# EthanD11/RS-VIO

Measured on AMD Instinct MI355X. Metric: stereo frames/sec (tracker+BA) on 752×480 EuRoC stream; BA ms/iter at window=10, higher is better.
Workload: dtype f32 (tracker) / f64 (BA)

## Files before the change

rs-vio_amd/csrc/pyramid.hip:

```cpp
#include "pyramid.hpp"

namespace rsvio {

namespace {

constexpr int TW = 64;
constexpr int TH = 8;
constexpr int STRIP_COLS = 320;
constexpr size_t LDS_CAP = 64 << 10;

__device__ __forceinline__ float triangle_kernel(float x) {
    float ax = fabsf(x);
    return ax < 1.0f ? 1.0f - ax : 0.0f;
}

__global__ void make_taps_kernel(TapTable tab, int n_entries) {
    int e = blockIdx.x * blockDim.x + threadIdx.x;
    if (e >= n_entries) return;
    int in_len = tab.ent_in_len[e];
    int out_len = tab.ent_out_len[e];
    int o = tab.ent_out_idx[e];
    float ratio = (float)in_len / (float)out_len;
    float sratio = ratio < 1.0f ? 1.0f : ratio;
    float support = 1.0f * sratio;
    float inputc = ((float)o + 0.5f) * ratio;
    long long left = (long long)floorf(inputc - support);
    if (left < 0) left = 0;
    if (left > (long long)in_len - 1) left = in_len - 1;
    long long right = (long long)ceilf(inputc + support);
    if (right < left + 1) right = left + 1;
    if (right > (long long)in_len) right = in_len;
    inputc = inputc - 0.5f;
    int cnt = (int)(right - left);
    float* w = tab.weights + (size_t)e * tab.max_taps;
    float sum = 0.0f;
    for (int k = 0; k < cnt; ++k) {
        float wv = triangle_kernel(((float)(left + k) - inputc) / sratio);
        w[k] = wv;
        sum += wv;
    }
    for (int k = 0; k < cnt; ++k) w[k] = w[k] / sum;
    tab.left[e] = (int)left;
    tab.count[e] = cnt;
}

__global__ __launch_bounds__(256) void pyramid_kernel(PyrLaunch L, PyrIO io) {
    extern __shared__ uint32_t smem[];
    const int img = blockIdx.y;
    {
        const int fb = (int)blockIdx.x - (L.copy_blocks + L.tile_start[L.levels]);
        if (fb >= 0) {
            if (img == 0 && fb < io.fast_cells) {
                const uint8_t* s0 = io.psrc ? io.psrc : io.src[0];
                fast_cell(s0, io.fg, fb, nullptr, nullptr, 0, io.fast_pt, io.fast_aff,
                          reinterpret_cast<uint8_t*>(smem));
            }
            return;
        }
    }
    const uint8_t* __restrict__ src = io.psrc ? io.psrc + (size_t)img * L.w * L.h : io.src[img];
    uint8_t* __restrict__ dst_base = io.psrc ? io.pdst + (size_t)img * L.pyr_bytes : io.dst[img];
    int b = blockIdx.x;
    const bool aligned = ((reinterpret_cast<uintptr_t>(src) | reinterpret_cast<uintptr_t>(dst_base)) & 15) == 0;
    if (b < L.copy_blocks) {
        const size_t tot = (size_t)L.w * L.h;
        if (!aligned) {
            for (size_t i = (size_t)b * blockDim.x + threadIdx.x; i < tot; i += (size_t)L.copy_blocks * blockDim.x)
                dst_base[i] = src[i];
            return;
        }
        const size_t n16 = tot / 16;
        const uint4* s4 = reinterpret_cast<const uint4*>(src);
        uint4* d4 = reinterpret_cast<uint4*>(dst_base);
        for (size_t i = (size_t)b * blockDim.x + threadIdx.x; i < n16; i += (size_t)L.copy_blocks * blockDim.x)
            d4[i] = s4[i];
        size_t tail0 = n16 * 16;
        if (b == 0)
            for (size_t i = tail0 + threadIdx.x; i < tot; i += blockDim.x) dst_base[i] = src[i];
        return;
    }
    b -= L.copy_blocks;
    int lev = 1;
    while (lev < L.levels - 1 && b >= L.tile_start[lev + 1]) ++lev;
    b -= L.tile_start[lev];
    const int nw = (int)level_w(L.w, lev), nh = (int)level_h(L.h, lev);
    const int tw = L.tile_w[lev], th = L.tile_h[lev];
    const int tiles_x = (nw + tw - 1) / tw;
    const int tx = b % tiles_x, ty = b / tiles_x;
    const int ox0 = tx * tw, ox1 = min(ox0 + tw, nw);
    const int oy0 = ty * th, oy1 = min(oy0 + th, nh);
    const int rows = oy1 - oy0, cols_out = ox1 - ox0;
    const int hx = L.hx_ent[lev], vy = L.vy_ent[lev];
    const TapTable& T = L.tab;
    const int xl = T.left[hx + ox0];
    const int xr = T.left[hx + ox1 - 1] + T.count[hx + ox1 - 1];
    const int yl = T.left[vy + oy0];
    const int yr = T.left[vy + oy1 - 1] + T.count[vy + oy1 - 1];
    const int ncols = xr - xl, nrows = yr - yl;
    const int xa = xl & ~3, xoff = xl - xa;
    const int pd = (xr - xa + 3) >> 2;
    const bool direct = (L.direct >> lev) & 1;
    uint8_t* strip = reinterpret_cast<uint8_t*>(smem);
    if (!direct) {
        if (aligned && (L.w & 3) == 0) {
            const uint32_t* s32 = reinterpret_cast<const uint32_t*>(src);
            const int wd = (int)(L.w >> 2);
            for (int idx = threadIdx.x; idx < nrows * pd; idx += blockDim.x) {
                const int r = idx / pd, d = idx - r * pd;
                smem[idx] = s32[(size_t)(yl + r) * wd + (xa >> 2) + d];
            }
        } else {
            for (int idx = threadIdx.x; idx < nrows * pd * 4; idx += blockDim.x) {
                const int r = idx / (pd * 4), c = idx - r * pd * 4;
                strip[idx] = (xa + c < (int)L.w) ? src[(size_t)(yl + r) * L.w + xa + c] : 0;
            }
        }
    }
    float* tmp = reinterpret_cast<float*>(smem + (direct ? 0 : nrows * pd));
    __syncthreads();
    for (int idx = threadIdx.x; idx < rows * ncols; idx += blockDim.x) {
        const int r = idx / ncols, c = idx - r * ncols;
        const int e = vy + oy0 + r;
        const int vl = T.left[e], vc = T.count[e];
        const float* __restrict__ vw = T.weights + (size_t)e * T.max_taps;
        float acc = 0.0f;
        if (!direct) {
            const uint8_t* col = strip + (vl - yl) * pd * 4 + xoff + c;
            for (int k = 0; k < vc; ++k) acc += (float)col[k * pd * 4] * vw[k];
        } else {
            const uint8_t* __restrict__ col = src + (size_t)vl * L.w + xl + c;
            for (int k = 0; k < vc; k += 8) {
                float px[8];
#pragma unroll
                for (int u = 0; u < 8; ++u) px[u] = (k + u < vc) ? (float)col[(size_t)(k + u) * L.w] : 0.0f;
#pragma unroll
                for (int u = 0; u < 8; ++u)
                    if (k + u < vc) acc += px[u] * vw[k + u];
            }
        }
        tmp[r * ncols + c] = acc;
    }
    __syncthreads();
    uint8_t* __restrict__ dst = dst_base + level_offset(L.w, L.h, lev);
    for (int idx = threadIdx.x; idx < rows * cols_out; idx += blockDim.x) {
        const int r = idx / cols_out, c = idx - r * cols_out;
        const int e = hx + ox0 + c;
        const int hl = T.left[e] - xl, hc = T.count[e];
        const float* __restrict__ hw = T.weights + (size_t)e * T.max_taps;
        const float* __restrict__ row = tmp + r * ncols + hl;
        float acc = 0.0f;
        for (int k = 0; k < hc; ++k) acc += row[k] * hw[k];
        float cl = acc < 0.0f ? 0.0f : (acc > 255.0f ? 255.0f : acc);
        dst[(size_t)(oy0 + r) * nw + ox0 + c] = (uint8_t)roundf(cl);
    }
}

}

void PyramidPlan::init(int w_, int h_, int levels_) {
    w = w_;
    h = h_;
    levels = levels_;
    if (levels < 1 || levels > kMaxLevels) throw std::invalid_argument("levels must be in [1, 8]");
    if (w < 16 || h < 16) throw std::invalid_argument("image too small");
    std::vector<int> in_len, out_len, out_idx;
    float max_ratio = 1.0f;
    memset(&launch, 0, sizeof(launch));
    for (int i = 1; i < levels; ++i) {
        int nw = (int)level_w(w, i), nh = (int)level_h(h, i);
        if (nw < 1 || nh < 1) throw std::invalid_argument("too many levels for image size");
        launch.hx_ent[i] = (int)in_len.size();
        for (int o = 0; o < nw; ++o) { in_len.push_back(w); out_len.push_back(nw); out_idx.push_back(o); }
        launch.vy_ent[i] = (int)in_len.size();
        for (int o = 0; o < nh; ++o) { in_len.push_back(h); out_len.push_back(nh); out_idx.push_back(o); }
        float rx = (float)w / nw, ry = (float)h / nh;
        max_ratio = std::max(max_ratio, std::max(rx, ry));
        launch.tile_h[i] = std::max(1, std::min(TH, (int)(16.0f / ry)));
        launch.tile_w[i] = std::max(1, std::min(TW, (int)std::floor((STRIP_COLS - 2.0f * rx - 4.0f) / rx)));
    }
    n_entries = (int)in_len.size();
    max_taps = (int)std::ceil(2.0f * max_ratio) + 4;
    int tiles = 0;
    for (int i = 1; i < levels; ++i) {
        launch.tile_start[i] = tiles;
        int nw = (int)level_w(w, i), nh = (int)level_h(h, i);
        tiles += ((nw + launch.tile_w[i] - 1) / launch.tile_w[i]) * ((nh + launch.tile_h[i] - 1) / launch.tile_h[i]);
    }
    launch.tile_start[levels] = tiles;
    launch.copy_blocks = std::max(1, (int)(((size_t)w * h / 16 + 255) / 256 / 4));
    total_blocks = launch.copy_blocks + tiles;
    launch.w = (uint32_t)w;
    launch.h = (uint32_t)h;
    launch.levels = levels;
    launch.pyr_bytes = level_offset(w, h, levels);
    if (n_entries > 0) {
        i_in.alloc(n_entries); i_out.alloc(n_entries); i_idx.alloc(n_entries);
        d_left.alloc(n_entries); d_count.alloc(n_entries);
        d_w.alloc((size_t)n_entries * max_taps);
        RSVIO_HIP(hipMemcpy(i_in.p, in_len.data(), sizeof(int) * n_entries, hipMemcpyHostToDevice));
        RSVIO_HIP(hipMemcpy(i_out.p, out_len.data(), sizeof(int) * n_entries, hipMemcpyHostToDevice));
        RSVIO_HIP(hipMemcpy(i_idx.p, out_idx.data(), sizeof(int) * n_entries, hipMemcpyHostToDevice));
        TapTable t;
        t.left = d_left.p; t.count = d_count.p; t.weights = d_w.p; t.max_taps = max_taps;
        t.ent_in_len = i_in.p; t.ent_out_len = i_out.p; t.ent_out_idx = i_idx.p;
        hipLaunchKernelGGL(make_taps_kernel, dim3((n_entries + 255) / 256), dim3(256), 0, 0, t, n_entries);
        RSVIO_HIP(hipGetLastError());
        RSVIO_HIP(hipDeviceSynchronize());
        launch.tab = t;
        std::vector<int> left(n_entries), count(n_entries);
        RSVIO_HIP(hipMemcpy(left.data(), d_left.p, sizeof(int) * n_entries, hipMemcpyDeviceToHost));
        RSVIO_HIP(hipMemcpy(count.data(), d_count.p, sizeof(int) * n_entries, hipMemcpyDeviceToHost));
        for (int i = 1; i < levels; ++i) {
            const int nw = (int)level_w(w, i), nh = (int)level_h(h, i);
            const int tw = launch.tile_w[i], th = launch.tile_h[i];
            size_t strip = 0, vert = 0;
            for (int ox0 = 0; ox0 < nw; ox0 += tw) {
                const int ox1 = std::min(ox0 + tw, nw);
                const int xl = left[launch.hx_ent[i] + ox0];
                const int xr = left[launch.hx_ent[i] + ox1 - 1] + count[launch.hx_ent[i] + ox1 - 1];
                const size_t pd = (size_t)(xr - (xl & ~3) + 3) / 4;
                for (int oy0 = 0; oy0 < nh; oy0 += th) {
                    const int oy1 = std::min(oy0 + th, nh);
                    const int yl = left[launch.vy_ent[i] + oy0];
                    const int yr = left[launch.vy_ent[i] + oy1 - 1] + count[launch.vy_ent[i] + oy1 - 1];
                    strip = std::max(strip, 4 * pd * (size_t)(yr - yl));
                    vert = std::max(vert, 4 * (size_t)(oy1 - oy0) * (size_t)(xr - xl));
                }
            }
            if (vert > LDS_CAP) throw std::invalid_argument("image too wide for the pyramid tile");
            if (strip + vert > LDS_CAP) launch.direct |= 1u << i;
            lds_bytes = std::max(lds_bytes, ((launch.direct >> i) & 1) ? vert : strip + vert);
        }
    }
}

void PyramidPlan::enqueue(const PyrIO& io, int n_img, hipStream_t s) const {
    if (n_img <= 0) return;
    if (n_img > (io.psrc ? 65535 : kMaxPyrIO)) throw std::invalid_argument("too many images per pyramid launch");
    const size_t lds = io.fast_cells > 0 ? std::max(lds_bytes, (size_t)io.fg.g * io.fg.g) : lds_bytes;
    hipLaunchKernelGGL(pyramid_kernel, dim3(total_blocks + std::max(io.fast_cells, 0), n_img), dim3(256), lds, s,
                       launch, io);
    RSVIO_HIP(hipGetLastError());
}

void PyramidPlan::enqueue(const uint8_t* d_imgs, int n_img, uint8_t* d_pyrs, hipStream_t s) const {
    for (int i0 = 0; i0 < n_img; i0 += 65535) {
        PyrIO io{};
        io.psrc = d_imgs + (size_t)i0 * w * h;
        io.pdst = d_pyrs + (size_t)i0 * pyr_bytes();
        enqueue(io, std::min(65535, n_img - i0), s);
    }
}

}
```

rs-vio_amd/csrc/pyramid.hpp:

```cpp
#pragma once
#include <algorithm>
#include <cmath>
#include <cstring>
#include <stdexcept>
#include <vector>

#include "common.hpp"
#include "fast.hpp"

namespace rsvio {

constexpr int kMaxLevels = 8;

struct TapTable {
    int* left = nullptr;
    int* count = nullptr;
    float* weights = nullptr;
    int max_taps = 0;
    const int* ent_in_len = nullptr;
    const int* ent_out_len = nullptr;
    const int* ent_out_idx = nullptr;
};

struct PyrLaunch {
    uint32_t w, h;
    int levels;
    size_t pyr_bytes;
    int copy_blocks;
    int tile_start[kMaxLevels + 1];
    int tile_w[kMaxLevels];
    int tile_h[kMaxLevels];
    uint32_t direct;
    int hx_ent[kMaxLevels];
    int vy_ent[kMaxLevels];
    TapTable tab;
};

constexpr int kMaxPyrIO = 8;
struct PyrIO {
    const uint8_t* src[kMaxPyrIO];
    uint8_t* dst[kMaxPyrIO];
    const uint8_t* psrc;
    uint8_t* pdst;
    int fast_cells;
    GridGeom fg;
    int4* fast_pt;
    float* fast_aff;
};

struct PyramidPlan {
    int w = 0, h = 0, levels = 0;
    int n_entries = 0, max_taps = 0, total_blocks = 0;
    size_t lds_bytes = 0;
    PyrLaunch launch;
    DevBuf<int> i_in, i_out, i_idx, d_left, d_count;
    DevBuf<float> d_w;
    void init(int w, int h, int levels);
    size_t pyr_bytes() const { return level_offset(w, h, levels); }
    void enqueue(const uint8_t* d_imgs, int n_img, uint8_t* d_pyrs, hipStream_t s) const;
    void enqueue(const PyrIO& io, int n_img, hipStream_t s) const;
};

}
```

Before: 4859.

## Stage tap weights in LDS and vectorize vertical pass over packed pixels

Reworks the pyramid downsample kernel. Tap tables are cached in LDS per tile, and tile bounds are computed inline rather than read from global memory. The vertical pass now processes four packed bytes per thread from the strip, strided index division is replaced with incremental DivStep counters, and global loads are unrolled to raise memory-level parallelism. The tile height default grows from 8 to 12 and the LDS sizing is updated, which raises LDS use per block and may lower occupancy.

```diff
diff --git a/rs-vio_amd/csrc/pyramid.hip b/rs-vio_amd/csrc/pyramid.hip
--- a/rs-vio_amd/csrc/pyramid.hip
+++ b/rs-vio_amd/csrc/pyramid.hip
@@ -4,22 +4,29 @@
 
 namespace {
 
+constexpr int NT = 256;
 constexpr int TW = 64;
-constexpr int TH = 8;
+#ifndef RSVIO_PYR_TH
+#define RSVIO_PYR_TH 12
+#endif
+constexpr int TH = RSVIO_PYR_TH;
 constexpr int STRIP_COLS = 320;
 constexpr size_t LDS_CAP = 64 << 10;
+constexpr int SU = 8;
+constexpr int WU = 4;
+static_assert(TW + TH <= NT, "one thread per tap row of a tile");
 
 __device__ __forceinline__ float triangle_kernel(float x) {
     float ax = fabsf(x);
     return ax < 1.0f ? 1.0f - ax : 0.0f;
 }
 
-__global__ void make_taps_kernel(TapTable tab, int n_entries) {
-    int e = blockIdx.x * blockDim.x + threadIdx.x;
-    if (e >= n_entries) return;
-    int in_len = tab.ent_in_len[e];
-    int out_len = tab.ent_out_len[e];
-    int o = tab.ent_out_idx[e];
+struct TapSpan {
+    int left, count;
+    float inputc, sratio;
+};
+
+__device__ __forceinline__ TapSpan tap_span(int in_len, int out_len, int o) {
     float ratio = (float)in_len / (float)out_len;
     float sratio = ratio < 1.0f ? 1.0f : ratio;
     float support = 1.0f * sratio;
@@ -31,18 +38,42 @@
     if (right < left + 1) right = left + 1;
     if (right > (long long)in_len) right = in_len;
     inputc = inputc - 0.5f;
-    int cnt = (int)(right - left);
+    return TapSpan{(int)left, (int)(right - left), inputc, sratio};
+}
+
+__global__ void make_taps_kernel(TapTable tab, int n_entries) {
+    int e = blockIdx.x * blockDim.x + threadIdx.x;
+    if (e >= n_entries) return;
+    const TapSpan sp = tap_span(tab.ent_in_len[e], tab.ent_out_len[e], tab.ent_out_idx[e]);
     float* w = tab.weights + (size_t)e * tab.max_taps;
     float sum = 0.0f;
-    for (int k = 0; k < cnt; ++k) {
-        float wv = triangle_kernel(((float)(left + k) - inputc) / sratio);
+    for (int k = 0; k < sp.count; ++k) {
+        float wv = triangle_kernel(((float)((long long)sp.left + k) - sp.inputc) / sp.sratio);
         w[k] = wv;
         sum += wv;
     }
-    for (int k = 0; k < cnt; ++k) w[k] = w[k] / sum;
-    tab.left[e] = (int)left;
-    tab.count[e] = cnt;
-}
+    for (int k = 0; k < sp.count; ++k) w[k] = w[k] / sum;
+    tab.left[e] = sp.left;
+    tab.count[e] = sp.count;
+}
+
+struct DivStep {
+    int q, r, dq, dr, n;
+    __device__ __forceinline__ explicit DivStep(int n_) : n(n_) {
+        q = (int)threadIdx.x / n;
+        r = (int)threadIdx.x - q * n;
+        dq = NT / n;
+        dr = NT - dq * n;
+    }
+    __device__ __forceinline__ void next() {
+        q += dq;
+        r += dr;
+        if (r >= n) {
+            r -= n;
+            ++q;
+        }
+    }
+};
 
 __global__ __launch_bounds__(256) void pyramid_kernel(PyrLaunch L, PyrIO io) {
     extern __shared__ uint32_t smem[];
@@ -92,62 +123,135 @@
     const int rows = oy1 - oy0, cols_out = ox1 - ox0;
     const int hx = L.hx_ent[lev], vy = L.vy_ent[lev];
     const TapTable& T = L.tab;
-    const int xl = T.left[hx + ox0];
-    const int xr = T.left[hx + ox1 - 1] + T.count[hx + ox1 - 1];
-    const int yl = T.left[vy + oy0];
-    const int yr = T.left[vy + oy1 - 1] + T.count[vy + oy1 - 1];
+    const int tid = threadIdx.x;
+    const TapSpan sx0 = tap_span((int)L.w, nw, ox0), sx1 = tap_span((int)L.w, nw, ox1 - 1);
+    const TapSpan sy0 = tap_span((int)L.h, nh, oy0), sy1 = tap_span((int)L.h, nh, oy1 - 1);
+    const int xl = sx0.left, xr = sx1.left + sx1.count;
+    const int yl = sy0.left, yr = sy1.left + sy1.count;
     const int ncols = xr - xl, nrows = yr - yl;
-    const int xa = xl & ~3, xoff = xl - xa;
+    const bool direct = (L.direct >> lev) & 1;
+    const int xa = direct ? xl : (xl & ~3);
     const int pd = (xr - xa + 3) >> 2;
-    const bool direct = (L.direct >> lev) & 1;
-    uint8_t* strip = reinterpret_cast<uint8_t*>(smem);
+    const int tc = L.tap_cap[lev];
+    const int ne = cols_out + rows, nwt = ne * tc;
+    float* tmp = reinterpret_cast<float*>(smem);
+    uint32_t* strip32 = smem + rows * 4 * pd;
+    uint8_t* strip = reinterpret_cast<uint8_t*>(strip32);
+    int* s_left = reinterpret_cast<int*>(strip32 + (direct ? 0 : nrows * pd));
+    int* s_count = s_left + ne;
+    float* s_w = reinterpret_cast<float*>(s_count + ne);
+    int t_left = 0, t_count = 0;
+    if (tid < ne) {
+        const int e = tid < cols_out ? hx + ox0 + tid : vy + oy0 + (tid - cols_out);
+        t_left = T.left[e];
+        t_count = T.count[e];
+    }
+    float wv[WU];
+    DivStep jk(tc);
+#pragma unroll
+    for (int u = 0; u < WU; ++u) {
+        const int j = jk.q;
+        const int e = j < cols_out ? hx + ox0 + j : vy + oy0 + (j - cols_out);
+        wv[u] = (tid + u * NT < nwt) ? T.weights[(size_t)e * T.max_taps + jk.r] : 0.0f;
+        jk.next();
+    }
     if (!direct) {
         if (aligned && (L.w & 3) == 0) {
-            const uint32_t* s32 = reinterpret_cast<const uint32_t*>(src);
-            const int wd = (int)(L.w >> 2);
-            for (int idx = threadIdx.x; idx < nrows * pd; idx += blockDim.x) {
-                const int r = idx / pd, d = idx - r * pd;
-                smem[idx] = s32[(size_t)(yl + r) * wd + (xa >> 2) + d];
+            const uint32_t* __restrict__ s32 = reinterpret_cast<const uint32_t*>(src);
+            const int wd = (int)(L.w >> 2), n = nrows * pd;
+            DivStep rd(pd);
+            for (int base = tid; base < n; base += NT * SU) {
+                uint32_t v[SU];
+#pragma unroll
+                for (int u = 0; u < SU; ++u) {
+                    v[u] = (base + u * NT < n) ? s32[(size_t)(yl + rd.q) * wd + (xa >> 2) + rd.r] : 0u;
+                    rd.next();
+                }
+#pragma unroll
+                for (int u = 0; u < SU; ++u)
+                    if (base + u * NT < n) strip32[base + u * NT] = v[u];
             }
         } else {
-            for (int idx = threadIdx.x; idx < nrows * pd * 4; idx += blockDim.x) {
-                const int r = idx / (pd * 4), c = idx - r * pd * 4;
-                strip[idx] = (xa + c < (int)L.w) ? src[(size_t)(yl + r) * L.w + xa + c] : 0;
-            }
-        }
-    }
-    float* tmp = reinterpret_cast<float*>(smem + (direct ? 0 : nrows * pd));
+            const int n = nrows * pd * 4;
+            DivStep rc(pd * 4);
+            for (int base = tid; base < n; base += NT * SU) {
+                uint8_t v[SU];
+#pragma unroll
+                for (int u = 0; u < SU; ++u) {
+                    v[u] = (base + u * NT < n && xa + rc.r < (int)L.w) ? src[(size_t)(yl + rc.q) * L.w + xa + rc.r]
+                                                                       : (uint8_t)0;
+                    rc.next();
+                }
+#pragma unroll
+                for (int u = 0; u < SU; ++u)
+                    if (base + u * NT < n) strip[base + u * NT] = v[u];
+            }
+        }
+    }
+    if (tid < ne) {
+        s_left[tid] = t_left;
+        s_count[tid] = t_count;
+    }
+#pragma unroll
+    for (int u = 0; u < WU; ++u)
+        if (tid + u * NT < nwt) s_w[tid + u * NT] = wv[u];
+    for (int idx = tid + WU * NT; idx < nwt; idx += NT) {
+        const int j = jk.q;
+        const int e = j < cols_out ? hx + ox0 + j : vy + oy0 + (j - cols_out);
+        s_w[idx] = T.weights[(size_t)e * T.max_taps + jk.r];
+        jk.next();
+    }
     __syncthreads();
-    for (int idx = threadIdx.x; idx < rows * ncols; idx += blockDim.x) {
-        const int r = idx / ncols, c = idx - r * ncols;
-        const int e = vy + oy0 + r;
-        const int vl = T.left[e], vc = T.count[e];
-        const float* __restrict__ vw = T.weights + (size_t)e * T.max_taps;
-        float acc = 0.0f;
-        if (!direct) {
-            const uint8_t* col = strip + (vl - yl) * pd * 4 + xoff + c;
-            for (int k = 0; k < vc; ++k) acc += (float)col[k * pd * 4] * vw[k];
-        } else {
-            const uint8_t* __restrict__ col = src + (size_t)vl * L.w + xl + c;
-            for (int k = 0; k < vc; k += 8) {
-                float px[8];
-#pragma unroll
-                for (int u = 0; u < 8; ++u) px[u] = (k + u < vc) ? (float)col[(size_t)(k + u) * L.w] : 0.0f;
-#pragma unroll
-                for (int u = 0; u < 8; ++u)
-                    if (k + u < vc) acc += px[u] * vw[k + u];
-            }
-        }
-        tmp[r * ncols + c] = acc;
+    if (!direct) {
+        DivStep rd(pd);
+        for (int idx = tid; idx < rows * pd; idx += NT, rd.next()) {
+            const int r = rd.q, d = rd.r, j = cols_out + r;
+            const int vc = s_count[j];
+            const float* vw = s_w + j * tc;
+            const uint32_t* col = strip32 + (s_left[j] - yl) * pd + d;
+            float a0 = 0.0f, a1 = 0.0f, a2 = 0.0f, a3 = 0.0f;
+            for (int k = 0; k < vc; ++k) {
+                const uint32_t p = col[k * pd];
+                const float wk = vw[k];
+                a0 += (float)(p & 0xffu) * wk;
+                a1 += (float)((p >> 8) & 0xffu) * wk;
+                a2 += (float)((p >> 16) & 0xffu) * wk;
+                a3 += (float)(p >> 24) * wk;
+            }
+            float* o = tmp + (r * pd + d) * 4;
+            o[0] = a0;
+            o[1] = a1;
+            o[2] = a2;
+            o[3] = a3;
+        }
+    } else {
+        for (int r = 0; r < rows; ++r) {
+            const int j = cols_out + r;
+            const int vl = s_left[j], vc = s_count[j];
+            const float* vw = s_w + j * tc;
+            for (int c = tid; c < ncols; c += NT) {
+                const uint8_t* __restrict__ col = src + (size_t)vl * L.w + xl + c;
+                float acc = 0.0f;
+                for (int k = 0; k < vc; k += 8) {
+                    float px[8];
+#pragma unroll
+                    for (int u = 0; u < 8; ++u) px[u] = (k + u < vc) ? (float)col[(size_t)(k + u) * L.w] : 0.0f;
+#pragma unroll
+                    for (int u = 0; u < 8; ++u)
+                        if (k + u < vc) acc += px[u] * vw[k + u];
+                }
+                tmp[r * pd * 4 + c] = acc;
+            }
+        }
     }
     __syncthreads();
     uint8_t* __restrict__ dst = dst_base + level_offset(L.w, L.h, lev);
-    for (int idx = threadIdx.x; idx < rows * cols_out; idx += blockDim.x) {
-        const int r = idx / cols_out, c = idx - r * cols_out;
-        const int e = hx + ox0 + c;
-        const int hl = T.left[e] - xl, hc = T.count[e];
-        const float* __restrict__ hw = T.weights + (size_t)e * T.max_taps;
-        const float* __restrict__ row = tmp + r * ncols + hl;
+    DivStep rc(cols_out);
+    for (int idx = tid; idx < rows * cols_out; idx += NT, rc.next()) {
+        const int r = rc.q, c = rc.r;
+        const int hc = s_count[c];
+        const float* hw = s_w + c * tc;
+        const float* row = tmp + r * pd * 4 + (s_left[c] - xa);
         float acc = 0.0f;
         for (int k = 0; k < hc; ++k) acc += row[k] * hw[k];
         float cl = acc < 0.0f ? 0.0f : (acc > 255.0f ? 255.0f : acc);
@@ -175,7 +279,7 @@
         for (int o = 0; o < nh; ++o) { in_len.push_back(h); out_len.push_back(nh); out_idx.push_back(o); }
         float rx = (float)w / nw, ry = (float)h / nh;
         max_ratio = std::max(max_ratio, std::max(rx, ry));
-        launch.tile_h[i] = std::max(1, std::min(TH, (int)(16.0f / ry)));
+        launch.tile_h[i] = std::max(1, std::min(TH, (int)(2.0f * TH / ry)));
         launch.tile_w[i] = std::max(1, std::min(TW, (int)std::floor((STRIP_COLS - 2.0f * rx - 4.0f) / rx)));
     }
     n_entries = (int)in_len.size();
@@ -213,23 +317,28 @@
         for (int i = 1; i < levels; ++i) {
             const int nw = (int)level_w(w, i), nh = (int)level_h(h, i);
             const int tw = launch.tile_w[i], th = launch.tile_h[i];
-            size_t strip = 0, vert = 0;
+            int tc = 1;
+            for (int e = launch.hx_ent[i]; e < launch.hx_ent[i] + nw + nh; ++e) tc = std::max(tc, count[e]);
+            launch.tap_cap[i] = tc;
+            size_t staged = 0, unstaged = 0;
             for (int ox0 = 0; ox0 < nw; ox0 += tw) {
                 const int ox1 = std::min(ox0 + tw, nw);
                 const int xl = left[launch.hx_ent[i] + ox0];
                 const int xr = left[launch.hx_ent[i] + ox1 - 1] + count[launch.hx_ent[i] + ox1 - 1];
-                const size_t pd = (size_t)(xr - (xl & ~3) + 3) / 4;
+                const size_t pd = (size_t)(xr - (xl & ~3) + 3) / 4, pdd = (size_t)(xr - xl + 3) / 4;
                 for (int oy0 = 0; oy0 < nh; oy0 += th) {
                     const int oy1 = std::min(oy0 + th, nh);
                     const int yl = left[launch.vy_ent[i] + oy0];
                     const int yr = left[launch.vy_ent[i] + oy1 - 1] + count[launch.vy_ent[i] + oy1 - 1];
-                    strip = std::max(strip, 4 * pd * (size_t)(yr - yl));
-                    vert = std::max(vert, 4 * (size_t)(oy1 - oy0) * (size_t)(xr - xl));
+                    const size_t rows = (size_t)(oy1 - oy0);
+                    const size_t taps = 4 * (rows + (size_t)(ox1 - ox0)) * (size_t)(tc + 2);
+                    staged = std::max(staged, 4 * pd * (size_t)(yr - yl) + 16 * rows * pd + taps);
+                    unstaged = std::max(unstaged, 16 * rows * pdd + taps);
                 }
             }
-            if (vert > LDS_CAP) throw std::invalid_argument("image too wide for the pyramid tile");
-            if (strip + vert > LDS_CAP) launch.direct |= 1u << i;
-            lds_bytes = std::max(lds_bytes, ((launch.direct >> i) & 1) ? vert : strip + vert);
+            if (unstaged > LDS_CAP) throw std::invalid_argument("image too wide for the pyramid tile");
+            if (staged > LDS_CAP) launch.direct |= 1u << i;
+            lds_bytes = std::max(lds_bytes, ((launch.direct >> i) & 1) ? unstaged : staged);
         }
     }
 }
diff --git a/rs-vio_amd/csrc/pyramid.hpp b/rs-vio_amd/csrc/pyramid.hpp
--- a/rs-vio_amd/csrc/pyramid.hpp
+++ b/rs-vio_amd/csrc/pyramid.hpp
@@ -33,6 +33,7 @@
     uint32_t direct;
     int hx_ent[kMaxLevels];
     int vy_ent[kMaxLevels];
+    int tap_cap[kMaxLevels];
     TapTable tab;
 };
 
```

Result: no change. 4932, median of 4 (+1.5%).
